# NVlabs/STEP

Measured on AMD Instinct MI355X. Metric: clips_per_sec_T32_224, higher is better.
Workload: dtype bf16; 1 GPU; C2: I3D backbone (BaseNet conv3d_1a..mixed_4f) forward, 8 x [3,32,224,224] clips per GPU, inputs resident in HBM, random-init weights; clips_per_gpu=8, T=32, HW=224, parallelism=clip-sharded replicas x1 (no data-path collective), batches_in_flight=2

## Files before the change

### include/step_amd.h

```cpp
#ifndef STEP_AMD_H
#define STEP_AMD_H

#include <stddef.h>
#include <stdint.h>

#ifdef __cplusplus
extern "C" {
#endif

#define STEP_API __attribute__((visibility("default")))

typedef void* step_stream_t;

enum { STEP_F32 = 0, STEP_BF16 = 1, STEP_F16 = 2 };
enum { STEP_NCHW = 0, STEP_NHWC = 1 };

enum {
    STEP_OK = 0,
    STEP_E_DTYPE = -1,
    STEP_E_SHAPE = -2,
    STEP_E_NULL = -3,
    STEP_E_UNSUPPORTED = -4,
    STEP_E_ALIGN = -5
};

STEP_API const char* step_version(void);
STEP_API int step_abi_version(void);

STEP_API int step_mfma_clock_probe(unsigned long long* out, int workgroups, int iters, step_stream_t stream);

STEP_API int step_clock_sample(unsigned long long* out, int workgroups, int ticks_100mhz, step_stream_t stream);

STEP_API int step_hbm_stream_probe(const void* src, void* dst, size_t bytes, int workgroups, step_stream_t stream);

enum {
    STEP_OPT_CONV_IMPL = 0,
    STEP_OPT_CONV_NB,
    STEP_OPT_CONV_WAVES,
    STEP_OPT_CONV_PHASED,
    STEP_OPT_CONV_GEN,
    STEP_OPT_CONV_GMODE,
    STEP_OPT_CONV_PWS,
    STEP_OPT_CONV_SPLITK,
    STEP_OPT_CONV_TAIL,
    STEP_OPT_CONV_SLOTS,
    STEP_OPT_POOL_DIRECT,
    STEP_OPT_WGRAD_MINPIX,
    STEP_OPT_WGRAD16_LDS,
    STEP_OPT_CONV_GROUP_PW,
    STEP_OPT_CLIP_VEC,
    STEP_OPT_CONV_NB_RULE,
    STEP_OPT_THROUGHPUT,
    STEP_OPT_CONV_PERSIST,
    STEP_OPT_CONV_PWS_WAVES,
    STEP_OPT_CONV_GROUP_NARROW,
    STEP_OPT_COUNT_
};
STEP_API int step_set_option(int option, int value);
STEP_API int step_get_option(int option, int* value);
STEP_API void step_reset_options(void);
STEP_API const char* step_option_name(int option);

STEP_API int step_roi_align_forward(const void* feat, int dtype, int layout, const float* rois, int K, int B,
                                    int C, int H, int W, int pooled_h, int pooled_w, float spatial_scale,
                                    int sampling_ratio, void* out, step_stream_t stream);

STEP_API int step_roi_align_tubes_forward(const void* feat, int dtype, const float* rois, int K, int B, int T_all, int T, int C,
                                          int H, int W, int pooled_h, int pooled_w, float spatial_scale, int sampling_ratio,
                                          void* out, step_stream_t stream);

#define STEP_ROI_BWD_GATHER 0
#define STEP_ROI_BWD_ATOMIC 1
STEP_API int step_roi_align_backward(const float* grad, int layout, const float* rois, int K, int B, int C, int H,
                                     int W, int pooled_h, int pooled_w, float spatial_scale, int sampling_ratio,
                                     int mode, float* grad_feat, step_stream_t stream);

STEP_API int step_roi_pool_forward(const void* feat, int dtype, int layout, const float* rois, int K, int B, int C,
                                   int H, int W, int pooled_h, int pooled_w, float spatial_scale, void* out,
                                   int32_t* argmax, step_stream_t stream);

STEP_API int step_roi_pool_backward(const float* grad, const int32_t* argmax, int layout, const float* rois, int K,
                                    int B, int C, int H, int W, int pooled_h, int pooled_w, float* grad_feat,
                                    step_stream_t stream);

STEP_API size_t step_nms_scratch_bytes(int G, int kmax);
STEP_API int step_nms_batched(const float* boxes, const float* scores, const int32_t* counts, int G, int kmax,
                              float threshold, uint8_t* keep, void* scratch, step_stream_t stream);
STEP_API int step_nms_batched_f64(const double* boxes, const double* scores, const int32_t* counts, int G, int kmax,
                                  float threshold, uint8_t* keep, void* scratch, step_stream_t stream);

STEP_API int step_detect_nms(const float* prob, long long prob_stride, int NC, const float* loc, long long loc_stride,
                             const int32_t* tube_start, const int32_t* tube_count, int B, int kmax, float conf_thresh,
                             float nms_thresh, float width, float height, uint8_t* keep, float* boxes_out, step_stream_t stream);

#define STEP_DETECT_ITERS_MAX 8
STEP_API int step_detect_compact(const uint8_t* keep, const float* const* boxes, const float* const* scores, const long long* score_strides,
                                 const int32_t* tube_start, int I, int B, int NC, int kmax, float width, float height, float* out_boxes,
                                 float* out_scores, long long* out_cls, long long* out_tube, int32_t* counts, step_stream_t stream);

STEP_API int step_detect_merge(const float* boxes, const int32_t* counts, const int32_t* order, const int32_t* sel_counts, int G, int cap,
                               float global_thresh, int32_t* cluster, int32_t* lead_pos, float* merged, int32_t* n_clusters,
                               step_stream_t stream);

STEP_API int step_round_sig4(const float* in, long long n, double* out, int32_t* status, step_stream_t stream);

STEP_API int step_eval_match(const double* det_boxes, const int32_t* det_cls, const long long* det_start, const double* gt_boxes,
                             const int32_t* gt_cls, const long long* gt_start, int NI, long long R, long long M, int gt_max, double thresh,
                             uint8_t* label, int32_t* match, step_stream_t stream);

STEP_API int step_eval_ap(const long long* cls_start, const uint8_t* label, const long long* num_gt, int NC, long long R, double* precision,
                          double* recall, double* ap, step_stream_t stream);

typedef struct step_conv_desc {
    int dtype;
    int N, D, H, W;
    int Cin, Cout;
    int kd, kh, kw;
    int x_cstride, x_coff;
    int y_cstride, y_coff;
    int res_cstride, res_coff;
    int relu;
    int split;
    int y2_cstride, y2_coff;
} step_conv_desc;

STEP_API size_t step_conv_packed_elems(int Cout, int Cin, int kd, int kh, int kw);
STEP_API int step_conv_pack_weight(const float* w, int Cout, int Cin, int kd, int kh, int kw, int dtype,
                                   const int32_t* perm_c, void* packed, step_stream_t stream);
STEP_API int step_conv_pack_weight_dgrad(const float* w, int Cout, int Cin, int kd, int kh, int kw, int dtype, int cin_pad,
                                         void* packed, step_stream_t stream);
typedef struct step_pack_item {
    const float* w;
    const int32_t* perm_c;
    void* packed;
    int Cout, Cin, w_cin, cin_lo;
    int kd, kh, kw;
    int dgrad, cin_pad;
    int reserved;
// ... 217 lines not shown
```

### step_amd/_capi.py

```python
import ctypes as C

F32, BF16, F16 = 0, 1, 2
NCHW, NHWC = 0, 1
ROI_BWD_GATHER, ROI_BWD_ATOMIC = 0, 1
ABI_VERSION = 42

vp, fp, ip, u8p = C.c_void_p, C.c_void_p, C.c_void_p, C.c_void_p
i, f, ll, sz = C.c_int, C.c_float, C.c_longlong, C.c_size_t


class ConvDesc(C.Structure):
    _fields_ = [(n, C.c_int) for n in (
        "dtype", "N", "D", "H", "W", "Cin", "Cout", "kd", "kh", "kw", "x_cstride", "x_coff", "y_cstride", "y_coff",
        "res_cstride", "res_coff", "relu", "split", "y2_cstride", "y2_coff")]


class PackItem(C.Structure):
    _fields_ = [("w", C.c_void_p), ("perm_c", C.c_void_p), ("packed", C.c_void_p)] + [(n, C.c_int) for n in (
        "Cout", "Cin", "w_cin", "cin_lo", "kd", "kh", "kw", "dgrad", "cin_pad", "reserved")]


class ConvItem(C.Structure):
    _fields_ = [("desc", C.POINTER(ConvDesc)), ("x", C.c_void_p), ("w_packed", C.c_void_p), ("scale", C.c_void_p), ("shift", C.c_void_p),
                ("res", C.c_void_p), ("y", C.c_void_p)]
# ... 46 lines not shown
    "step_conv_forward_pre_pool": (i, [C.POINTER(ConvDesc), vp, vp, fp, fp, vp, fp, fp, i, vp, vp, sz, vp]),
    "step_conv_forward_pre_pool_tiles": (i, [C.POINTER(ConvDesc), vp, vp, fp, fp, vp, fp, fp, i, vp, vp, sz, vp]),
    "step_conv_pre_pool_finish": (i, [C.POINTER(ConvDesc), vp, vp, sz, vp]),
    "step_conv_wgrad": (i, [C.POINTER(ConvDesc), vp, fp, fp, i, vp]),
    "step_conv_wgrad_workspace_bytes": (sz, [C.POINTER(ConvDesc)]),
    "step_conv_wgrad_ws": (i, [C.POINTER(ConvDesc), vp, fp, fp, i, vp, sz, vp]),
    "step_conv_wgrad16": (i, [C.POINTER(ConvDesc), vp, vp, fp, i, vp]),
    "step_conv_wgrad16_workspace_bytes": (sz, [C.POINTER(ConvDesc)]),
    "step_conv_wgrad16_ws": (i, [C.POINTER(ConvDesc), vp, vp, fp, i, vp, sz, vp]),
    "step_conv_wgrad_kernel_name": (i, [C.POINTER(ConvDesc), i, C.c_char_p, i]),
    "step_conv_wgrad_partial": (i, [C.POINTER(ConvDesc), vp, vp, i, fp, i, vp, sz, C.POINTER(WgradReduceItem), vp]),
    "step_wgrad_reduce_group": (i, [C.POINTER(WgradReduceItem), i, vp]),
    "step_conv_forward_ws": (i, [C.POINTER(ConvDesc), vp, vp, fp, fp, vp, vp, vp, vp, sz, vp]),
    "step_conv_kernel_name": (i, [C.POINTER(ConvDesc), C.c_char_p, i]),
    "step_conv_plan_info": (i, [C.POINTER(ConvDesc), C.POINTER(C.c_int), i]),
    "step_conv_pre_pool_plan_info": (i, [C.POINTER(ConvDesc), C.POINTER(C.c_int), i]),
    "step_stem_packed_elems": (sz, [i]),
    "step_stem_pack_weight": (i, [fp, i, i, vp, vp]),
    "step_stem_forward": (i, [i, vp, i, i, i, i, vp, fp, fp, i, i, vp, i, i, vp]),
    "step_stem_pool_workspace_bytes": (sz, [i, i, i, i, i, i]),
    "step_stem_pool_forward": (i, [i, vp, i, i, i, i, vp, fp, fp, i, vp, i, i, vp, sz, vp]),
    "step_stem_pool_forward_tiles": (i, [i, vp, i, i, i, i, vp, fp, fp, i, vp, i, i, vp, sz, vp]),
    "step_stem_pool_finish": (i, [i, vp, i, i, i, i, i, vp, i, i, vp, sz, vp]),
    "step_stem_pool_forward_u8": (i, [i, vp, i, i, i, i, i, C.POINTER(C.c_float), C.POINTER(C.c_float), vp, fp, fp, i, vp, i, i, vp, sz, vp]),
    "step_stem_kernel_name": (i, [i, C.c_char_p, i]),
    "step_stem_wgrad": (i, [i, vp, i, i, i, i, fp, i, fp, i, vp]),
    "step_stem_wgrad_workspace_bytes": (sz, [i, i, i, i, i]),
    "step_stem_wgrad_ws": (i, [i, vp, i, i, i, i, fp, i, fp, i, vp, sz, vp]),
    "step_stem_wgrad16_workspace_bytes": (sz, [i, i, i, i, i, i]),
    "step_stem_wgrad16": (i, [i, vp, i, i, i, i, vp, i, fp, i, vp, sz, vp]),
    "step_pool_out_size": (i, [i, i, i]),
    "step_maxpool3d_tf": (i, [i, vp, i, i, i, i, i, i, i, i, i, i, i, i, i, vp, i, i, vp]),
    "step_maxpool3d_tf_backward": (i, [i, vp, i, i, i, i, i, i, i, i, i, i, i, i, i, fp, fp, vp]),
    "step_maxpool3d_tf_backward_gather": (i, [i, vp, i, i, i, i, i, i, i, i, i, i, i, i, i, i, vp, i, vp, u8p, vp]),
    "step_clip_from_u8": (i, [vp, i, i, i, i, i, C.POINTER(C.c_float), C.POINTER(C.c_float), i, vp, vp]),
    "step_clip_augment_u8": (i, [vp, i, i, i, i, i, C.POINTER(C.c_float), C.POINTER(C.c_float), i, i, vp, vp]),
    "step_avgpool_hw": (i, [i, vp, i, i, i, i, i, i, i, vp, vp]),
    "step_transpose_cs": (i, [vp, i, vp, i, i, i, ll, i, vp]),
    "step_act_grad": (i, [i, vp, i, i, vp, i, fp, ll, i, i, fp, vp, vp]),
    "step_bn_train_workspace_bytes": (sz, [ll, i]),
    "step_bn_train_forward": (i, [i, vp, i, ll, i, fp, fp, f, f, fp, fp, fp, fp, i, vp, i, vp, sz, vp]),
    "step_bn_train_backward": (i, [i, vp, i, vp, i, i, vp, i, ll, i, i, fp, fp, fp, vp, fp, fp, vp, sz, vp]),
    "step_head_outputs": (i, [i, vp, i, vp, i, i, i, i, i, fp, fp, fp, fp, fp, fp, fp, fp, fp, vp]),
    "step_head_outputs_backward": (i, [i, vp, i, vp, i, i, i, i, i, fp, fp, fp, fp, fp, vp, vp, vp]),
    "step_dropout_forward": (i, [i, vp, vp, vp, ll, C.c_double, vp, vp]),
    "step_dropout_backward": (i, [i, vp, vp, vp, ll, C.c_double, vp]),
    "step_rng_words": (i, [vp, C.c_ulonglong, ll, vp, vp]),
    "step_tube_update": (i, [fp, i, i, fp, fp, fp, i, i, i, ip, i, f, f, fp, fp, fp, fp, vp]),
    "step_select_prepare": (i, [fp, fp, fp, fp, i, i, i, i, ip, fp, ip, i, f, f, fp, fp, fp, fp, fp, vp]),
    "step_select_train": (i, [fp, fp, fp, fp, fp, i, i, i, i, ip, i, i, fp, ip, i, i, fp, vp, i, i, i, i, f, f, i, i, i, i, fp, fp, fp, fp, ip, vp]),
    "step_adam_flat": (i, [fp, fp, fp, fp, ll, vp, fp, fp, i, C.c_double, C.c_double, C.c_double, i, f, i, vp]),
    "step_adam_flat_dev": (i, [fp, fp, fp, fp, ll, vp, fp, fp, i, C.c_double, C.c_double, C.c_double, vp, fp, f, i, vp]),
    "step_adam_flat_amp": (i, [fp, fp, fp, fp, ll, vp, fp, fp, i, C.c_double, C.c_double, C.c_double, vp, fp, f, i, fp, f, f, i, vp]),
    "step_sgd_flat": (i, [fp, fp, fp, ll, vp, fp, fp, i, C.c_double, C.c_double, i, i, f, i, vp]),
    "step_sgd_flat_dev": (i, [fp, fp, fp, ll, vp, fp, fp, i, C.c_double, C.c_double, i, vp, f, i, vp]),
    "step_sgd_flat_amp": (i, [fp, fp, fp, ll, vp, fp, fp, i, C.c_double, C.c_double, i, vp, f, i, fp, f, f, i, vp]),
    "step_grad_pack16": (i, [i, fp, fp, vp, ll, f, vp]),
    "step_grad_unpack16": (i, [i, vp, fp, ll, vp]),
}


def declare(lib, strict=True):
    for name, (res, args) in SIGNATURES.items():
        if not strict and not hasattr(lib, name):
            continue
        fn = getattr(lib, name)
        fn.restype = res
        fn.argtypes = args
    return lib


_ERR = {-1: "unsupported dtype", -2: "bad shape", -3: "null pointer", -4: "unsupported configuration",
        -5: "misaligned pointer or channel count"}


def check(status, what):
    if status != 0:
        msg = _ERR.get(status, "hipError_t %d" % status) if status < 0 else "hipError_t %d" % status
        raise RuntimeError("%s failed: %s" % (what, msg))


OPTION_IDS = {name: k for k, name in enumerate((
    "conv_impl", "conv_nb", "conv_waves", "conv_phased", "conv_gen", "conv_gmode", "conv_pws", "conv_splitk", "conv_tail",
    "conv_slots", "pool_direct", "wgrad_minpix", "wgrad16_lds", "conv_group_pw", "clip_vec", "conv_nb_rule", "throughput", "conv_persist", "conv_pws_waves", "conv_group_narrow"))}


def set_option(lib, name, value):
    check(lib.step_set_option(OPTION_IDS[name], int(value)), "step_set_option(%s, %r)" % (name, value))


def get_option(lib, name):
    v = C.c_int()
    check(lib.step_get_option(OPTION_IDS[name], C.byref(v)), "step_get_option(%s)" % name)
    return v.value


class options:

    def __init__(self, lib, **kw):
        self.lib, self.kw = lib, kw

    def __enter__(self):
        self.prev = {k: get_option(self.lib, k) for k in self.kw}
        for k, v in self.kw.items():
            set_option(self.lib, k, v)
        return self

    def __exit__(self, *exc):
        for k, v in self.prev.items():
            set_option(self.lib, k, v)
        return False
```

### step_amd/csrc/conv_igemm.hip

```cpp
#include "conv_common.h"

namespace step {

template <typename T, int TWL, int NB, int KD, int KH, int KW, bool FLAT, int CKT>
__global__ __launch_bounds__(256) void conv_igemm_kernel(ConvParams p) {
    constexpr int TW = 1 << TWL, TH = 128 >> TWL;
    constexpr int HH_ = TH + KH - 1, HW_ = TW + KW - 1;
    constexpr int NPIX = FLAT ? 128 : KD * HH_ * HW_;
    constexpr int ES = (int)sizeof(T);
    constexpr int VEC = 16 / ES;
    constexpr int PITCH = CKT * ES;
    constexpr int KSTEPS = CKT / 16;
    constexpr int SLOTS = PITCH / 16;
    constexpr int PPR = (16 / SLOTS) > 0 ? (16 / SLOTS) : 1;
    constexpr int NTAPS = KD * KH * KW;
    constexpr int NVEC = NPIX * SLOTS;
    constexpr int ITER = (NVEC + 255) / 256;
    typedef typename Ld16<T>::type vec16;
    typedef typename frag<T>::type frag_t;

    constexpr int LDSB = (NPIX * PITCH > 16384) ? NPIX * PITCH : 16384;
    __shared__ __attribute__((aligned(16))) unsigned char lds[LDSB];

    const int tid = threadIdx.x;
// ... 219 lines not shown
        }
    } else if (co < Cout && ci < Cin && tap < ntaps) {
        const int cs = cin_lo + (perm ? perm[ci] : ci);
        v = w[((size_t)co * w_cin + cs) * ntaps + tap];
    }
    return v;
}

template <typename T, bool DGRAD>
__global__ void pack_weight_kernel(const float* __restrict__ w, const int32_t* __restrict__ perm, T* __restrict__ out,
                                   int Cout, int Cin, int ntaps, int KC16, long long total, int Cw) {
    for (long long idx = (long long)blockIdx.x * blockDim.x + threadIdx.x; idx < total;
         idx += (long long)blockDim.x * gridDim.x)
        out[idx] = elem<T>::from_f32(pack_value<DGRAD>(w, perm, idx, Cout, Cin, ntaps, KC16, Cw, DGRAD ? Cout : Cin, 0));
}

template <typename T>
__global__ void pack_weights_kernel(const step_pack_item* __restrict__ items) {
    const step_pack_item it = items[blockIdx.y];
    const int ntaps = it.kd * it.kh * it.kw;
    const int pc_out = it.dgrad ? it.Cin : it.Cout, pc_in = it.dgrad ? it.cin_pad : it.Cin;
    const int KC16 = (pc_in + CK - 1) / CK * 2;
    const long long total = (long long)((pc_out + 31) / 32) * taps_padded(ntaps) * KC16 * 512;
    T* out = (T*)it.packed;
    if (it.dgrad) {
        for (long long idx = (long long)blockIdx.x * blockDim.x + threadIdx.x; idx < total; idx += (long long)blockDim.x * gridDim.x)
            out[idx] = elem<T>::from_f32(pack_value<true>(it.w, it.perm_c, idx, pc_out, pc_in, ntaps, KC16, it.Cout, it.w_cin, it.cin_lo));
    } else {
        for (long long idx = (long long)blockIdx.x * blockDim.x + threadIdx.x; idx < total; idx += (long long)blockDim.x * gridDim.x)
            out[idx] = elem<T>::from_f32(pack_value<false>(it.w, it.perm_c, idx, pc_out, pc_in, ntaps, KC16, 0, it.w_cin, it.cin_lo));
    }
}


template <typename T, int TWL, int KD, int KH, int KW, bool FLAT, int CKT>
static int launch_nb(const ConvParams& p, int NB, dim3 grid, step_stream_t stream) {
    switch (NB) {
        case 1: STEP_LAUNCH((conv_igemm_kernel<T, TWL, 1, KD, KH, KW, FLAT, CKT>), grid, dim3(256), stream, p); break;
        case 2: STEP_LAUNCH((conv_igemm_kernel<T, TWL, 2, KD, KH, KW, FLAT, CKT>), grid, dim3(256), stream, p); break;
        case 3: STEP_LAUNCH((conv_igemm_kernel<T, TWL, 3, KD, KH, KW, FLAT, CKT>), grid, dim3(256), stream, p); break;
        default: STEP_LAUNCH((conv_igemm_kernel<T, TWL, 4, KD, KH, KW, FLAT, CKT>), grid, dim3(256), stream, p); break;
    }
    return STEP_LAUNCH_CHECK();
}

static int pick_nb(int nblk32, long long mtiles) {
    int best = 1;
    long long best_cost = -1;
    const int cand[4] = {4, 3, 2, 1};
    for (int k = 0; k < 4; ++k) {
        const int nb = cand[k];
        const long long groups = ceil_div(nblk32, nb);
        const long long wgs = groups * mtiles;
        const long long cost = ceil_div64(wgs, 1024) * (nb + 2) * 8 - nb;
        if (best_cost < 0 || cost < best_cost) { best_cost = cost; best = nb; }
    }
    return best;
}



static int pick_nb_tap(int nblk32, long long mtiles, int slots = 256) {
    const int forced = opt(STEP_OPT_CONV_NB);
    if (forced >= 1 && forced <= 3) return forced;
    int best = 1;
    double best_cost = -1;
    for (int nb = 3; nb >= 1; --nb) {
        const long long groups = ceil_div(nblk32, 2 * nb);
        const long long wgs = groups * mtiles;
        const double cost = opt(STEP_OPT_CONV_NB_RULE) == 1 ? (double)wgs * (2.0 * nb + 1.5) - 0.01 * nb
                                                            : (double)ceil_div64(wgs, slots) * (2.0 * nb + 1.5) - 0.01 * nb;
        if (best_cost < 0 || cost < best_cost) { best_cost = cost; best = nb; }
    }
    return best;
}


static step_conv_desc canonical_desc(const step_conv_desc* d) {
    step_conv_desc e = *d;
    if (e.kd == 1 && (long long)e.N * e.D <= 0x7fffffffLL) { e.D *= e.N; e.N = 1; }
    return e;
}

static long long best_gen_box(int D, int H, int W, int kd, int npix_limit, int* btd, int* bth, int* btw, int pxmax = 256) {
    long long best = -1; int bhalo = 0;
    for (int kw_ = 1; kw_ <= 8; ++kw_) {
        const int tw = ceil_div(W, kw_);
        if (tw > pxmax) continue;
        if (kw_ > 2 && tw < 16) break;
        for (int kh_ = 1; kh_ <= H; ++kh_) {
            const int th = ceil_div(H, kh_);
            if (th * tw > pxmax) continue;
            if (kh_ > 1 && th == ceil_div(H, kh_ - 1)) continue;
            for (int td = 1; td <= D && td * th * tw <= pxmax; ++td) {
                const int halo = (td + kd - 1) * (th + 2) * (tw + 2);
                if (halo > npix_limit) break;
                const long long tiles = (long long)ceil_div(D, td) * ceil_div(H, th) * ceil_div(W, tw);
                if (best < 0 || tiles < best || (tiles == best && halo < bhalo)) { best = tiles; bhalo = halo; *btd = td; *bth = th; *btw = tw; }
            }
        }
    }
    return best;
}

static bool prefer_four_waves(const ConvPlan& p8, const ConvPlan& p4, const step_conv_desc* d) {
    (void)p4;
    const long long wgs8 = p8.mtiles * ceil_div(ceil_div(d->Cout, 32), 2 * p8.NB);
    return wgs8 < 64;
}

static bool prefer_four_waves_pw(const step_conv_desc* d, long long wgs8) {
    const long long M = (long long)d->N * d->D * d->H * d->W;
    return wgs8 < 128 || M >= 65536;
}

static int gen_gmode(int td, int th, int tw, int tile_px) {
    if (opt(STEP_OPT_CONV_GMODE) == 0) return 0;
    const int spr = (tw + 15) / 16;
    if ((tw & 15) < 12) return 0;
    return td * th * spr <= tile_px / 16 ? 1 : 0;
}

static ConvPlan conv_plan(const step_conv_desc* d, bool allow_pws = true, int force_waves = 0, bool no_gen = false) {
    ConvPlan pl;
    pl.ok = true; pl.wide = false; pl.tiles_h = pl.tiles_w = 0; pl.impl = 0; pl.tps = 1; pl.mb = 2; pl.wv = 8; pl.ph = 0; pl.deep = false; pl.twl = 4; pl.tiles_d = d->D; pl.gtd = pl.gth = pl.gtw = 1; pl.gmode = 0; pl.ksplit = 0; pl.kchunk16 = 0; pl.mbk = 0; pl.mpad = 0; pl.cpad = 0;
    const int nblk32 = ceil_div(d->Cout, 32);
    const bool k1 = d->kd == 1 && d->kh == 1 && d->kw == 1;
    const bool k333 = d->kd == 3 && d->kh == 3 && d->kw == 3;
    const bool k133 = d->kd == 1 && d->kh == 3 && d->kw == 3;
    pl.flat = k1;
    if (k1) {
        pl.mtiles = ceil_div64((long long)d->N * d->D * d->H * d->W, 128);
        pl.NB = pick_nb(nblk32, pl.mtiles);
        const long long mt256 = ceil_div64((long long)d->N * d->D * d->H * d->W, 256);
        const int ov1 = conv_impl_override();
        {
            const int pws_env = opt(STEP_OPT_CONV_PWS);
            const int KC16 = ceil_div(d->Cin, CK) * 2;
            const long long M = (long long)d->N * d->D * d->H * d->W;
            const bool can = d->dtype != STEP_F32 && (d->Cin % 8) == 0 && (d->x_cstride % 8) == 0 && (d->x_coff % 8) == 0 && KC16 <= 16 &&
                             (d->y_cstride % 8) == 0 && (d->y_coff % 8) == 0 && (d->Cout % 8) == 0 && (d->res_cstride % 8) == 0 && (d->res_coff % 8) == 0 &&
                             (d->split == 0 || ((d->split % 8) == 0 && (d->y2_cstride % 8) == 0 && (d->y2_coff % 8) == 0)) && M >= 1024;
            const bool wins = d->res_cstride == 0 ? (KC16 >= 12 && nblk32 >= 6 && M >= 65536) : (KC16 >= 12 && nblk32 >= 16 && M >= 49152);
            if (allow_pws && can && pws_env != 0 && (pws_env == 1 || wins) && ov1 == -1) {
                int nbmax = 152 / (ceil_div(KC16, 4) * 4);
                if (nbmax > 16) nbmax = 16;
                if (nbmax > nblk32) nbmax = nblk32;
                const int groups = ceil_div(nblk32, nbmax);
                pl.impl = 4;
                pl.NB = ceil_div(nblk32, groups);
                pl.wv = 8;
                long long gx = 256 / groups;
                if (gx < 1) gx = 1;
                const long long need = ceil_div64(ceil_div64(M, 32), 8);
                if (gx > need) gx = need;
                pl.mtiles = gx;
                return pl;
            }
        }
        if (ov1 == 5 || (ov1 != 0 && d->Cin >= 128 && d->Cout >= 64 && mt256 * ceil_div(nblk32, 2) >= 32)) {
            pl.impl = 2;
            const int waves_env = opt(STEP_OPT_CONV_WAVES);
            const long long wgs8 = mt256 * ceil_div(nblk32, 2 * pick_nb_tap(nblk32, mt256));
            const bool four = waves_env == 4 || (waves_env != 8 && prefer_four_waves_pw(d, wgs8));
            pl.wv = four ? 4 : 8;
            pl.mtiles = four ? ceil_div64((long long)d->N * d->D * d->H * d->W, 128) : mt256;
            pl.NB = pick_nb_tap(nblk32, pl.mtiles, four ? 512 : 256);
            return pl;
        }
        const bool splitk_ok = opt(STEP_OPT_CONV_SPLITK) != 0;
        const long long M = (long long)d->N * d->D * d->H * d->W;
        if (splitk_ok && ov1 != 0 && d->Cin >= 512 && (d->Cin % 8) == 0 && (M <= 1024 || (M <= 4096 && d->Cout < 64)) && pl.mtiles * nblk32 < 64) {
            pl.impl = 3;
            pl.mbk = M <= 32 ? 1 : (M <= 64 ? 2 : 4);
            const int KC16 = ceil_div(d->Cin, CK) * 2;
            const long long mt = ceil_div64(M, pl.mbk * 32);
            int ks = (int)(512 / (mt * nblk32));
            if (ks < 1) ks = 1;
            pl.kchunk16 = ceil_div(KC16, ks);
            if (pl.kchunk16 < 8) pl.kchunk16 = 8;
            pl.ksplit = ceil_div(KC16, pl.kchunk16);
            pl.mpad = (int)(mt * pl.mbk * 32);
            pl.cpad = nblk32 * 32;
            pl.mtiles = mt;
            pl.NB = 1;
            return pl;
        }
        pl.deep = d->Cin >= 256;
        return pl;
    }
    if (!k333 && !k133) { pl.ok = false; pl.mtiles = 0; pl.NB = 1; return pl; }
    const int ov = conv_impl_override();
    const long long t16 = (long long)d->D * ceil_div(d->H, 16) * ceil_div(d->W, 16);
    const long long t32 = (long long)d->D * ceil_div(d->H, 8) * ceil_div(d->W, 32);
    const long long t8 = (long long)ceil_div(d->D, 4) * ceil_div(d->H, 8) * ceil_div(d->W, 8);
    int twl = 4;
    long long tbest = t16;
    if (t32 < tbest) { tbest = t32; twl = 5; }
    if (t8 < tbest) { tbest = t8; twl = 3; }
    int gtd = 1, gth = 1, gtw = 1;
    const int gen_pct = no_gen ? 0 : opt(STEP_OPT_CONV_GEN);
    const int twl_p2 = twl;
    const long long tbest_p2 = tbest;
    if (gen_pct > 0) {
        const long long tg = best_gen_box(d->D, d->H, d->W, d->kd, CONV_GEN_NPIX, &gtd, &gth, &gtw);
        if (tg > 0 && tg * 100 <= tbest * gen_pct) { tbest = tg; twl = 0; }
        if (twl == 0 && pick_nb_tap(nblk32, (long long)d->N * tbest) == 1) {
            int std_ = 1, sth = 1, stw = 1;
            const long long ts = best_gen_box(d->D, d->H, d->W, d->kd, CONV_GEN_NPIX_SMALL, &std_, &sth, &stw);
            if (ts > 0 && ts * 100 <= tbest_p2 * gen_pct && pick_nb_tap(nblk32, (long long)d->N * ts) == 1) {
                tbest = ts; gtd = std_; gth = sth; gtw = stw;
            } else {
                tbest = tbest_p2; twl = twl_p2;
            }
        }
    }
    const long long mt256 = (long long)d->N * tbest;
    const int waves_env = force_waves ? force_waves : opt(STEP_OPT_CONV_WAVES);
    ConvPlan p4 = pl;
    bool have4 = false;
    {
        const long long a16 = (long long)d->D * ceil_div(d->H, 8) * ceil_div(d->W, 16);
        const long long a32 = (long long)d->D * ceil_div(d->H, 4) * ceil_div(d->W, 32);
        const long long a8 = (long long)ceil_div(d->D, 2) * ceil_div(d->H, 8) * ceil_div(d->W, 8);
        int tw4 = 4;
        long long tb4 = a16;
        if (a8 < tb4) { tb4 = a8; tw4 = 3; }
        if (a32 * 100 < tb4 * 90) { tb4 = a32; tw4 = 5; }
        int g4d = 1, g4h = 1, g4w = 1;
        if (gen_pct > 0) {
            int limit = CONV_GEN_NPIX4_WIDE;
            for (int pass = 0; pass < 2; ++pass) {
                int td_ = 1, th_ = 1, tw_ = 1;
                const long long tg = best_gen_box(d->D, d->H, d->W, d->kd, limit, &td_, &th_, &tw_, 128);
                if (!(tg > 0 && tg * 100 <= tb4 * gen_pct)) break;
                const int nb = pick_nb_tap(nblk32, (long long)d->N * tg, 512);
                if (nb >= 3 && limit != CONV_GEN_NPIX4) { limit = CONV_GEN_NPIX4; continue; }
                tb4 = tg; tw4 = 0; g4d = td_; g4h = th_; g4w = tw_;
                break;
            }
        }
        p4.wv = 4; p4.twl = tw4; p4.wide = tw4 == 5; p4.gtd = g4d; p4.gth = g4h; p4.gtw = g4w;
        p4.gmode = tw4 == 0 ? gen_gmode(g4d, g4h, g4w, 128) : 0;
        if (tw4 == 0) {
            p4.tiles_d = ceil_div(d->D, g4d); p4.tiles_h = ceil_div(d->H, g4h); p4.tiles_w = ceil_div(d->W, g4w);
        } else {
            p4.tiles_d = tw4 == 3 ? ceil_div(d->D, 2) : d->D;
            p4.tiles_h = tw4 == 5 ? ceil_div(d->H, 4) : ceil_div(d->H, 8);
            p4.tiles_w = tw4 == 4 ? ceil_div(d->W, 16) : (tw4 == 5 ? ceil_div(d->W, 32) : ceil_div(d->W, 8));
        }
        p4.mtiles = (long long)d->N * tb4;
        p4.NB = pick_nb_tap(nblk32, p4.mtiles, 512);
        if (tw4 == 0 && p4.NB >= 3 && (g4d + d->kd - 1) * (g4h + 2) * (g4w + 2) > CONV_GEN_NPIX4) p4.NB = 2;
        p4.impl = 1; p4.tps = p4.NB == 1 ? 2 : 1; p4.mb = 2;
        have4 = true;
    }
    const bool fits32 = ((unsigned long long)d->N * d->D * d->H * d->W + 1) * (unsigned long long)d->x_cstride < 0xffffffffULL;
    const bool use_tap = fits32 && (ov >= 1 || (ov != 0 && (d->Cin >= 64 || mt256 >= 32)));
    if (use_tap) {
        pl.impl = 1;
        pl.tps = (ov == 1) ? 1 : 2;
        pl.mb = 2;
        pl.twl = twl;
        pl.wide = twl == 5;
        pl.gtd = gtd; pl.gth = gth; pl.gtw = gtw;
        pl.gmode = twl == 0 ? gen_gmode(gtd, gth, gtw, 256) : 0;
        if (twl == 0) {
            pl.tiles_d = ceil_div(d->D, gtd); pl.tiles_h = ceil_div(d->H, gth); pl.tiles_w = ceil_div(d->W, gtw);
        } else {
            pl.tiles_d = twl == 3 ? ceil_div(d->D, 4) : d->D;
            pl.tiles_h = twl == 4 ? ceil_div(d->H, 16) : ceil_div(d->H, 8);
            pl.tiles_w = twl == 4 ? ceil_div(d->W, 16) : (twl == 5 ? ceil_div(d->W, 32) : ceil_div(d->W, 8));
        }
        pl.mtiles = mt256;
        pl.NB = pick_nb_tap(nblk32, pl.mtiles);
        if (d->dtype != STEP_F32 && pl.tps == 2 && k333) {
            pl.ph = opt(STEP_OPT_CONV_PHASED) ? 1 : 0;
        }
        if (d->dtype != STEP_F32 && pl.tps == 2 && k133 && pl.twl == 0 && pl.NB <= 2 && opt(STEP_OPT_CONV_PHASED) == 2) pl.ph = 1;
        if (have4 && ov != 1 && (waves_env == 4 || (waves_env != 8 && prefer_four_waves(pl, p4, d)))) return p4;
        return pl;
    }
    const long long w16 = (long long)ceil_div(d->H, 8) * ceil_div(d->W, 16);
    const long long w32 = (long long)ceil_div(d->H, 4) * ceil_div(d->W, 32);
    pl.wide = w32 < w16;
    pl.tiles_h = pl.wide ? ceil_div(d->H, 4) : ceil_div(d->H, 8);
    pl.tiles_w = pl.wide ? ceil_div(d->W, 32) : ceil_div(d->W, 16);
    pl.mtiles = (long long)d->N * d->D * pl.tiles_h * pl.tiles_w;
    pl.NB = pick_nb(nblk32, pl.mtiles);
    return pl;
}


static inline void conv_set_box_magic(ConvParams& p, int kh, int kw) {
    const unsigned long long hw = (unsigned long long)(p.gtw + kw - 1), hhw = hw * (unsigned long long)(p.gth + kh - 1);
    p.mag_hw = (unsigned)((0x100000000ULL + hw - 1) / hw);
    p.mag_hhw = (unsigned)((0x100000000ULL + hhw - 1) / hhw);
}

template <typename T>
static int conv_forward_t(const step_conv_desc* d, ConvParams p, void* ws, size_t ws_bytes, step_stream_t stream) {
    constexpr int VEC = elem<T>::VEC;
    if (d->Cin % VEC || d->x_cstride % VEC || d->x_coff % VEC) return STEP_E_ALIGN;
    if (((uintptr_t)p.x % 16) || ((uintptr_t)p.w % 16)) return STEP_E_ALIGN;
    ConvPlan pl = conv_plan(d, p.x2 == nullptr, 0, p.pool_row != nullptr && p.pool_p2);
    if (!pl.ok) return STEP_E_UNSUPPORTED;
    if (p.x2 && pl.impl != 2) return STEP_E_UNSUPPORTED;
    if (p.x2 && pl.wv == 8 && pl.NB == 3) pl.NB = 2;
    if (pl.impl == 3) {
        const size_t need = (size_t)pl.ksplit * pl.mpad * pl.cpad * sizeof(float);
        if (ws && ws_bytes >= need && ((uintptr_t)ws % 16) == 0) return conv_splitk_launch<T>(pl, p, (float*)ws, stream);
        pl.impl = 0; pl.mtiles = ceil_div64(p.Mtot, 128); pl.NB = pick_nb(p.nblk32, pl.mtiles); pl.deep = d->Cin >= 256;
    }
    p.tiles_h = pl.tiles_h; p.tiles_w = pl.tiles_w; p.tiles_d = pl.tiles_d;
    p.gtd = pl.gtd; p.gth = pl.gth; p.gtw = pl.gtw; p.gmode = pl.gmode;
    conv_set_box_magic(p, d->kh, d->kw);
    auto grid1d = [&](int groups) {
        p.gx = (int)pl.mtiles; p.gy = groups;
        const long long tot = pl.mtiles * groups;
        p.gbase = 0; p.gcount = (int)((tot + 7) / 8 * 8);
        p.gpersist = 0;
        const long long slots_ = opt(STEP_OPT_CONV_SLOTS) > 0 ? opt(STEP_OPT_CONV_SLOTS) : 256;
        if (opt(STEP_OPT_CONV_PERSIST) != 0 && groups == 1 && pl.impl == 1 && pl.ph == 1 && pl.NB == 3 && p.pre_w && p.pool_row && tot > slots_)
            p.gpersist = (int)(slots_ / 8 * 8 > 0 ? slots_ / 8 * 8 : 8);
        return dim3((unsigned)p.gcount);
    };
    if (pl.impl == 4) {
        if (p.vec_epi && (!p.res || ((p.r_cstride % 8) == 0 && (p.r_coff % 8) == 0 && ((uintptr_t)p.res % 16) == 0)))
            return conv_pws_launch<T>(pl.NB, p, dim3((unsigned)pl.mtiles, (unsigned)ceil_div(p.nblk32, pl.NB)), stream);
        pl = conv_plan(d, false);
    }
    if (pl.impl == 2) {
        dim3 grid = grid1d(ceil_div(p.nblk32, 2 * pl.NB));
        return conv_pw_launch<T>(pl.NB, pl.wv, p, grid, stream);
    }
    if (pl.impl == 1) {
        const int groups = ceil_div(p.nblk32, 2 * pl.NB);
        const long long slots = opt(STEP_OPT_CONV_SLOTS) > 0 ? opt(STEP_OPT_CONV_SLOTS) : 256;
        const long long tail = pl.mtiles % slots;
        const bool tail_ok = opt(STEP_OPT_CONV_TAIL) != 0;
        const int tgroups = ceil_div(p.nblk32, 2);
        const bool box_ok = pl.twl != 0 || (pl.gtd + d->kd - 1) * (pl.gth + d->kh - 1) * (pl.gtw + d->kw - 1) <= conv_gen_npix(8, 1);
        if (tail_ok && box_ok && pl.wv == 8 && groups == 1 && pl.NB > 1 && pl.mtiles > slots && tail > 0 && tail * 4 <= slots && tail * tgroups <= slots) {
            const long long all = pl.mtiles;
            pl.mtiles = all - tail;
            dim3 grid = grid1d(1);
            int rc = conv_tap_launch<T>(pl, p, d->kd, grid, stream);
            if (rc != STEP_OK) return rc;
            ConvPlan pt = pl;
// ... 632 lines not shown
```

### step_amd/csrc/conv_tap_kernel.h

```cpp
#pragma once
#include "conv_common.h"
#include "conv_pw_kernel.h"

namespace step {


typedef short s16x8_pool __attribute__((ext_vector_type(8)));
#define NTAPS_EVEN_STEPS(KD, KH, KW, TPS) (((taps_padded((KD) * (KH) * (KW)) / (TPS)) & 1) == 0)

template <typename T, int TWL, int NB, int KD, int KH, int KW, int TPS, int MB, int WV, int PH = 0, bool GRP = false, bool PRE = false, bool POOL = false, bool PERSIST = false, int EXTB = 0>
__device__ __forceinline__ void conv_tap_body(const ConvParams& p, unsigned char* arena = nullptr) {
    static_assert(!PERSIST || (PH == 1 && !GRP && (NTAPS_EVEN_STEPS(KD, KH, KW, TPS))), "the persistent tile loop exists for the two-phase form with an even number of steps per slab");
    static_assert(!(PERSIST && POOL) || PRE, "persistent + pooled epilogue: the pooled tile lives in halo + stash (PRE)");
    static_assert(!POOL || (TWL == 3 && WV == 8 && PH == 1 && !GRP && sizeof(T) == 2 && KD == 3), "the pooled epilogue exists for the 4-plane 8x8 tile of the two-phase 16-bit form");
    static_assert(MB == 2 && (WV == 8 || WV == 4), "two accumulator rows per wave; 8 or 4 waves");
    static_assert(!PRE || (PH == 1 && sizeof(T) == 2), "the fused pointwise input exists for the two-phase 16-bit form");
    static_assert(PH == 0 || (WV == 8 && TPS == 2 && sizeof(T) == 2), "two-phase form: 8 waves, two taps per step, 16-bit storage");
    constexpr int NT = WV * 64;
    constexpr int WM = WV / 2;
    constexpr int TPXM = WM * MB * 32;
    constexpr bool GEN = (TWL == 0);
    constexpr int TDL = (TWL == 3) ? (TPXM == 256 ? 2 : 1) : 0;
    constexpr int THC = GEN ? 1 : (TPXM >> (TWL + TDL));
    constexpr int THL = GEN ? 0 : (THC == 16 ? 4 : (THC == 8 ? 3 : 2));
    const int TD = GEN ? p.gtd : (1 << TDL);
    const int TW = GEN ? p.gtw : (1 << TWL), TH = GEN ? p.gth : THC;
    const int TPX = TD * TH * TW;
    constexpr int HWPAD = (TWL == 3) ? 2 : 0;
    const int HH_ = TH + KH - 1, HWV = TW + KW - 1, HW_ = HWV + HWPAD;
    const int PD = TD + KD - 1;
    const int NPIX = PD * HH_ * HW_;
    constexpr int NPIX_MAX = GEN ? conv_gen_npix(WV, NB) : ((1 << TDL) + KD - 1) * (THC + KH - 1) * ((1 << TWL) + KW - 1 + HWPAD);
    constexpr int ES = (int)sizeof(T);
    constexpr int VEC = 16 / ES;
    constexpr int CKT = 64 / ES;
    constexpr int KS = CKT / 16;
    constexpr int PITCH = 80, SLOTS = 4;
    constexpr int NTAPS = KD * KH * KW;
    const int NVEC = NPIX * SLOTS;
    constexpr int ITER = (NPIX_MAX * SLOTS + NT - 1) / NT;
    constexpr int FRAGB = 512 * ES;
    constexpr int FRAGV = FRAGB / 16;
    constexpr int NBT = 2 * NB;
    constexpr int BTILE = NBT * KS * FRAGB;
    constexpr int BVEC = BTILE / 16;
    constexpr int Q = (BVEC + NT - 1) / NT;
    constexpr int NTP = taps_padded(NTAPS);
    constexpr int SPS = (TPS == 1) ? NTAPS : NTP / TPS;
    constexpr bool PADB = BVEC > NT && (BVEC % NT) != 0 && (NPIX_MAX * PITCH + 3 * TPS * Q * NT * 16) <= 160 * 1024;
    constexpr int BPITCH = PADB ? Q * NT * 16 : BTILE;
    constexpr int BSTEP = TPS * BPITCH;
    typedef typename Ld16<T>::type vec16;
    typedef typename frag<T>::type frag_t;

    constexpr bool TR = (ES == 2);
    constexpr int SS_BYTES = TR ? NBT * 32 * 2 * 4 : 0;
    constexpr int BBYTES = PH ? 2 * 2 * TPS * (NB * KS * FRAGB) : 3 * BSTEP;
    constexpr int STASH_BYTES = PRE ? NPIX_MAX * 64 : 0;
    constexpr int LDS_BYTES = NPIX_MAX * PITCH + BBYTES + SS_BYTES + STASH_BYTES;
    static_assert(LDS_BYTES <= 160 * 1024, "LDS budget");
    static_assert(!POOL || PERSIST || TPXM * (NBT * 64 + 16) <= NPIX_MAX * PITCH + BBYTES, "the pooled epilogue's tile lives in the halo / weight rings, below the scale table");
    static_assert(!POOL || !PERSIST || TPXM * (NBT * 64 + 16) <= NPIX_MAX * PITCH + STASH_BYTES, "persistent form: the pooled tile lives in halo + stash");
    static_assert(EXTB == 0 || EXTB >= LDS_BYTES, "the caller's arena holds this body");
    unsigned char* lds;
    if constexpr (EXTB != 0) {
        lds = arena;
    } else {
        __shared__ __attribute__((aligned(16))) unsigned char own[LDS_BYTES];
        lds = own;
    }
    unsigned char* const ldsA = lds;
    unsigned char* const ldsB = lds + NPIX_MAX * PITCH + (PERSIST ? STASH_BYTES + SS_BYTES : 0);
    float* const ldsS = (float*)(lds + NPIX_MAX * PITCH + (PERSIST ? STASH_BYTES : BBYTES));
    unsigned char* const ldsP = lds + NPIX_MAX * PITCH + (PERSIST ? 0 : BBYTES + SS_BYTES);
    auto tile_pix = [&](int m, int& td, int& th, int& tw) -> bool {
        if (GEN) {
            if (p.gmode) {
                const int pl_ = m & 31, blk = m >> 5;
                int g, j;
                if (pl_ < 4) { g = 0; j = pl_; }
                else if (pl_ < 12) { g = 1; j = pl_ - 4; }
                else if (pl_ < 16) { g = 0; j = pl_ - 8; }
                else if (pl_ < 20) { g = 1; j = pl_ - 8; }
                else if (pl_ < 28) { g = 0; j = pl_ - 12; }
                else { g = 1; j = pl_ - 16; }
                const int spr = (TW + 15) >> 4;
                const int slot = blk * 2 + g;
                const int row = slot / spr, col = (slot % spr) * 16 + j;
                const bool ok = row < TD * TH && col < TW;
                const int rc = row < TD * TH ? row : 0;
                tw = col; th = rc % TH; td = rc / TH;
                return ok;
            }
            const int mc = m < TPX ? m : 0;
            tw = mc % TW; const int q = mc / TW; th = q % TH; td = q / TH;
            return m < TPX;
        } else {
            td = m >> (TWL + THL); th = (m >> TWL) & (TH - 1); tw = m & (TW - 1);
            return true;
        }
    };

    auto tile_col = [](int th, int j) {
        if (TWL == 4) return (th & 1) ? ((j + 14) & 15) : j;
        if (TWL == 3) return (((th & 3) == 1) || ((th & 3) == 2)) ? (j ^ 4) : j;
        return j;
    };
    int tid = threadIdx.x;
    int lane = tid & 63;
#ifdef STEP_EMUL
    int wave = tid >> 6;
#else
    int wave = __builtin_amdgcn_readfirstlane(tid >> 6);
#endif
    int khalf = lane >> 5;
    int wm = (PH == 2) ? (wave >> 1) : (wave % WM), wn = (PH == 2) ? (wave & 1) : (wave / WM);
    auto relaunder = [&]() {
#ifndef STEP_EMUL
        asm volatile("" : "+v"(tid));
        asm volatile("" : "+s"(wave));
#endif
        lane = tid & 63; khalf = lane >> 5;
        wm = (PH == 2) ? (wave >> 1) : (wave % WM); wn = (PH == 2) ? (wave & 1) : (wave / WM);
    };

    int gbx, gby;
    unsigned vid = blockIdx.x - (unsigned)p.gbase;
    if constexpr (PERSIST) {
        while (vid < (unsigned)p.gcount && !grid_coords_of(p, vid, gbx, gby)) vid += gridDim.x;
        if (vid >= (unsigned)p.gcount) return;
    } else {
        if (!grid_coords(p, gbx, gby)) return;
    }
    STEP_PROBE_IDS(p);
    STEP_PROBE_MARK(p, 0);
    struct TileC { int tw_i, th_i, d0, n, h0, w0; };
    auto tile_of = [&](int bx) {
        TileC c;
        int t = bx + p.tile0;
        c.tw_i = t % p.tiles_w; t /= p.tiles_w;
        c.th_i = t % p.tiles_h; t /= p.tiles_h;
        c.d0 = (t % p.tiles_d) * TD;
        c.n = t / p.tiles_d;
        c.h0 = c.th_i * TH; c.w0 = c.tw_i * TW;
        return c;
    };
    TileC tc = tile_of(gbx);
    int tw_i = tc.tw_i, th_i = tc.th_i, d0 = tc.d0, n = tc.n, h0 = tc.h0, w0 = tc.w0;
    const int HHW = HH_ * HW_;
    const int nb0 = gby * NBT;
    const int KC16 = p.nchunks32 * 2;
    const int nslab = (p.Cin + CKT - 1) / CKT;
    const int S = nslab * SPS;

    const T* xg = (const T*)p.x;
    const unsigned char* wg = (const unsigned char*)p.w;

    const unsigned char* abase[MB];
#pragma unroll
    for (int mb = 0; mb < MB; ++mb) {
        const int m = wm * (MB * 32) + mb * 32 + (lane & 31);
        int td_, th_, tw_;
        tile_pix(m, td_, th_, tw_);
        abase[mb] = ldsA + ((td_ * HH_ + th_) * HW_ + tile_col(th_, tw_)) * PITCH + khalf * (ES == 4 ? 32 : 16);
    }

    f32x16 acc[MB][NB];
#pragma unroll
    for (int mb = 0; mb < MB; ++mb)
#pragma unroll
// ... 906 lines not shown
```

### step_amd/csrc/options.hip

```cpp
#include <atomic>
#include <limits.h>

#include "options.h"

namespace step {

namespace {
struct OptSpec { const char* name; int def, lo, hi; };
constexpr OptSpec SPEC[STEP_OPT_COUNT_] = {
    {"conv_impl", -1, -1, 5},
    {"conv_nb", 0, 0, 3},
    {"conv_waves", 0, 0, 8},
    {"conv_phased", 2, 0, 2},
    {"conv_gen", 93, 0, 100},
    {"conv_gmode", 1, 0, 1},
    {"conv_pws", -1, -1, 1},
    {"conv_splitk", 1, 0, 1},
    {"conv_tail", 1, 0, 1},
    {"conv_slots", 0, 0, 1 << 20},
    {"pool_direct", 0, 0, 1},
    {"wgrad_minpix", 0, 0, 1 << 24},
    {"wgrad16_lds", 1, 0, 2},
    {"conv_group_pw", 1 << 20, 0, 1 << 20},
    {"clip_vec", 1, 0, 1},
    {"conv_nb_rule", 0, 0, 1},
    {"throughput", 0, 0, 1},
    {"conv_persist", 1, 0, 1},
    {"conv_pws_waves", 0, 0, 16},
    {"conv_group_narrow", 1, 0, 2},
};
std::atomic<int> g_delta[STEP_OPT_COUNT_];
}

int opt(int id) { return SPEC[id].def + g_delta[id].load(std::memory_order_relaxed); }

}

using namespace step;

extern "C" {

int step_set_option(int option, int value) {
    if (option < 0 || option >= STEP_OPT_COUNT_) return STEP_E_SHAPE;
    if (value < SPEC[option].lo || value > SPEC[option].hi) return STEP_E_SHAPE;
    if (option == STEP_OPT_CONV_WAVES && value != 0 && value != 4 && value != 8) return STEP_E_SHAPE;
    if (option == STEP_OPT_CONV_PWS_WAVES && value != 0 && value != 8 && value != 16) return STEP_E_SHAPE;
    if (option == STEP_OPT_CONV_IMPL && (value == 3 || value == 4)) return STEP_E_SHAPE;
    g_delta[option].store(value - SPEC[option].def, std::memory_order_relaxed);
    return STEP_OK;
}

int step_get_option(int option, int* value) {
    if (option < 0 || option >= STEP_OPT_COUNT_) return STEP_E_SHAPE;
    if (!value) return STEP_E_NULL;
    *value = opt(option);
    return STEP_OK;
}

void step_reset_options(void) {
    for (int i = 0; i < STEP_OPT_COUNT_; ++i) g_delta[i].store(0, std::memory_order_relaxed);
}

const char* step_option_name(int option) {
    return (option < 0 || option >= STEP_OPT_COUNT_) ? nullptr : SPEC[option].name;
}

}
```

Measured before the change: 7433 clips/s.

## Add quad-width generic tile boxes for 3x3x3 bf16 convs with gmode 2 pixel mapping

Adds a new tile search that considers boxes of width 4 in W, stacking up to four depth slices into each 16-pixel MFMA row group, for 3x3x3 non-fp32 convolutions. A new gmode value maps lanes to (depth, h, w) inside the tap kernel, and a conv_gbox option (on by default) picks the quad box when it yields fewer tiles. The goal is to cut tile count and wasted padding on small spatial layers deep in the I3D stack. In exchange the halo per output pixel grows because the tiles are narrow, and the new mapping only applies on the 8-wave bf16 path.

```diff
diff --git a/include/step_amd.h b/include/step_amd.h
--- a/include/step_amd.h
+++ b/include/step_amd.h
@@ -54,6 +54,7 @@
     STEP_OPT_CONV_PERSIST,
     STEP_OPT_CONV_PWS_WAVES,
     STEP_OPT_CONV_GROUP_NARROW,
+    STEP_OPT_CONV_GBOX,
     STEP_OPT_COUNT_
 };
 STEP_API int step_set_option(int option, int value);
diff --git a/step_amd/_capi.py b/step_amd/_capi.py
--- a/step_amd/_capi.py
+++ b/step_amd/_capi.py
@@ -152,7 +152,7 @@
 
 OPTION_IDS = {name: k for k, name in enumerate((
     "conv_impl", "conv_nb", "conv_waves", "conv_phased", "conv_gen", "conv_gmode", "conv_pws", "conv_splitk", "conv_tail",
-    "conv_slots", "pool_direct", "wgrad_minpix", "wgrad16_lds", "conv_group_pw", "clip_vec", "conv_nb_rule", "throughput", "conv_persist", "conv_pws_waves", "conv_group_narrow"))}
+    "conv_slots", "pool_direct", "wgrad_minpix", "wgrad16_lds", "conv_group_pw", "clip_vec", "conv_nb_rule", "throughput", "conv_persist", "conv_pws_waves", "conv_group_narrow", "conv_gbox"))}
 
 
 def set_option(lib, name, value):
diff --git a/step_amd/csrc/conv_igemm.hip b/step_amd/csrc/conv_igemm.hip
--- a/step_amd/csrc/conv_igemm.hip
+++ b/step_amd/csrc/conv_igemm.hip
@@ -325,7 +325,7 @@
     return e;
 }
 
-static long long best_gen_box(int D, int H, int W, int kd, int npix_limit, int* btd, int* bth, int* btw, int pxmax = 256) {
+static long long best_gen_box(int D, int H, int W, int kd, int npix_limit, int* btd, int* bth, int* btw, int pxmax = 256, int* bquad = nullptr) {
     long long best = -1; int bhalo = 0;
     for (int kw_ = 1; kw_ <= 8; ++kw_) {
         const int tw = ceil_div(W, kw_);
@@ -343,6 +343,22 @@
             }
         }
     }
+    if (bquad) {
+        *bquad = 0;
+        const int mode = opt(STEP_OPT_CONV_GBOX);
+        if (mode != 0 && kd == 3 && pxmax == 256) {
+            long long qbest = -1; int qhalo = 0, qd = 1, qh = 4;
+            for (int th = 4; th <= 16; th += 4) {
+                for (int td = 1; td <= D && th * ceil_div(td, 4) <= 16; ++td) {
+                    const int halo = (td + kd - 1) * (th + 2) * 6;
+                    if (halo > npix_limit) break;
+                    const long long tiles = (long long)ceil_div(D, td) * ceil_div(H, th) * ceil_div(W, 4);
+                    if (qbest < 0 || tiles < qbest || (tiles == qbest && halo < qhalo)) { qbest = tiles; qhalo = halo; qd = td; qh = th; }
+                }
+            }
+            if (qbest > 0 && (mode == 2 || best < 0 || qbest < best)) { best = qbest; *btd = qd; *bth = qh; *btw = 4; *bquad = 1; }
+        }
+    }
     return best;
 }
 
@@ -357,8 +373,9 @@
     return wgs8 < 128 || M >= 65536;
 }
 
-static int gen_gmode(int td, int th, int tw, int tile_px) {
+static int gen_gmode(int td, int th, int tw, int tile_px, bool quad = false) {
     if (opt(STEP_OPT_CONV_GMODE) == 0) return 0;
+    if (quad) return 2;
     const int spr = (tw + 15) / 16;
     if ((tw & 15) < 12) return 0;
     return td * th * spr <= tile_px / 16 ? 1 : 0;
@@ -441,20 +458,22 @@
     long long tbest = t16;
     if (t32 < tbest) { tbest = t32; twl = 5; }
     if (t8 < tbest) { tbest = t8; twl = 3; }
-    int gtd = 1, gth = 1, gtw = 1;
+    int gtd = 1, gth = 1, gtw = 1, gquad = 0;
     const int gen_pct = no_gen ? 0 : opt(STEP_OPT_CONV_GEN);
     const int twl_p2 = twl;
     const long long tbest_p2 = tbest;
     if (gen_pct > 0) {
-        const long long tg = best_gen_box(d->D, d->H, d->W, d->kd, CONV_GEN_NPIX, &gtd, &gth, &gtw);
-        if (tg > 0 && tg * 100 <= tbest * gen_pct) { tbest = tg; twl = 0; }
+        const bool quad_ok = d->dtype != STEP_F32 && k333;
+        const bool quad_force = opt(STEP_OPT_CONV_GBOX) == 2;
+        const long long tg = best_gen_box(d->D, d->H, d->W, d->kd, CONV_GEN_NPIX, &gtd, &gth, &gtw, 256, quad_ok ? &gquad : nullptr);
+        if (tg > 0 && (tg * 100 <= tbest * gen_pct || (gquad && quad_force))) { tbest = tg; twl = 0; }
         if (twl == 0 && pick_nb_tap(nblk32, (long long)d->N * tbest) == 1) {
-            int std_ = 1, sth = 1, stw = 1;
-            const long long ts = best_gen_box(d->D, d->H, d->W, d->kd, CONV_GEN_NPIX_SMALL, &std_, &sth, &stw);
-            if (ts > 0 && ts * 100 <= tbest_p2 * gen_pct && pick_nb_tap(nblk32, (long long)d->N * ts) == 1) {
-                tbest = ts; gtd = std_; gth = sth; gtw = stw;
+            int std_ = 1, sth = 1, stw = 1, squad = 0;
+            const long long ts = best_gen_box(d->D, d->H, d->W, d->kd, CONV_GEN_NPIX_SMALL, &std_, &sth, &stw, 256, quad_ok ? &squad : nullptr);
+            if (ts > 0 && (ts * 100 <= tbest_p2 * gen_pct || (squad && quad_force)) && pick_nb_tap(nblk32, (long long)d->N * ts) == 1) {
+                tbest = ts; gtd = std_; gth = sth; gtw = stw; gquad = squad;
             } else {
-                tbest = tbest_p2; twl = twl_p2;
+                tbest = tbest_p2; twl = twl_p2; gquad = 0;
             }
         }
     }
@@ -507,7 +526,7 @@
         pl.twl = twl;
         pl.wide = twl == 5;
         pl.gtd = gtd; pl.gth = gth; pl.gtw = gtw;
-        pl.gmode = twl == 0 ? gen_gmode(gtd, gth, gtw, 256) : 0;
+        pl.gmode = twl == 0 ? gen_gmode(gtd, gth, gtw, 256, gquad != 0) : 0;
         if (twl == 0) {
             pl.tiles_d = ceil_div(d->D, gtd); pl.tiles_h = ceil_div(d->H, gth); pl.tiles_w = ceil_div(d->W, gtw);
         } else {
diff --git a/step_amd/csrc/conv_tap_kernel.h b/step_amd/csrc/conv_tap_kernel.h
--- a/step_amd/csrc/conv_tap_kernel.h
+++ b/step_amd/csrc/conv_tap_kernel.h
@@ -84,8 +84,14 @@
                 else if (pl_ < 20) { g = 1; j = pl_ - 8; }
                 else if (pl_ < 28) { g = 0; j = pl_ - 12; }
                 else { g = 1; j = pl_ - 16; }
+                const int slot = blk * 2 + g;
+                if (WV == 8 && ES == 2 && p.gmode == 2) {
+                    const int sq = slot / TH;
+                    const int d_ = 4 * sq + (j >> 2);
+                    tw = j & 3; th = slot - sq * TH; td = d_ < TD ? d_ : 0;
+                    return d_ < TD && tw < TW;
+                }
                 const int spr = (TW + 15) >> 4;
-                const int slot = blk * 2 + g;
                 const int row = slot / spr, col = (slot % spr) * 16 + j;
                 const bool ok = row < TD * TH && col < TW;
                 const int rc = row < TD * TH ? row : 0;
diff --git a/step_amd/csrc/options.hip b/step_amd/csrc/options.hip
--- a/step_amd/csrc/options.hip
+++ b/step_amd/csrc/options.hip
@@ -28,6 +28,7 @@
     {"conv_persist", 1, 0, 1},
     {"conv_pws_waves", 0, 0, 16},
     {"conv_group_narrow", 1, 0, 2},
+    {"conv_gbox", 1, 0, 2},
 };
 std::atomic<int> g_delta[STEP_OPT_COUNT_];
 }
```

Result: no change. 7476 clips/s, median of 2 (+0.6%).
